# evergreen-ci/evergreen

Measured on NVIDIA H100. Metric: tasks scheduled/sec over N distros; host-allocator decisions/sec at 1/2/4/8 GPU, higher is better.
Workload: dtype int64

## Files before the change

evergreen_b200/csrc/evg_plan_general.cuh:

```cuda
#pragma once

constexpr int kGTile = 2048;

struct DGen {
  int64_t n_tiles;
  int64_t tile0;
  const int32_t* tile_distro;
  const int64_t* tile_start;
  const int64_t* dtile_off;
  unsigned long long* vmm;
  uint32_t* key_lo[2];
  uint32_t* key_hi[2];
  uint32_t* idx[2];
  uint32_t* e;
  uint32_t* tile_sum;
  uint32_t* tile_hist;
  uint4* wl;
  struct URec* pay;
  unsigned int* ccount;
  uint4* tie;
  int32_t* maxpass;
  uint32_t* run;
  uint32_t* pown;
  uint32_t* pver;
  uint32_t* pedge;
  uint32_t* sedge;
  uint32_t* rank;
  unsigned int* rcount;
  uint2* blist;
  unsigned int* bcount;
  uint4* usum;
  uint2* hlist;
  unsigned int* hcount;
  int64_t* tv;
};

__device__ __forceinline__ int gen_bits(const DGen& G, int d) {
  const unsigned long long r = G.vmm[2 * d] - G.vmm[2 * d + 1];
  return r == 0 ? 0 : 64 - __clzll((long long)r);
}
__device__ __forceinline__ int gen_npass(int bits) { return (bits + 7) >> 3; }

struct __align__(16) URec {
  int32_t prio, nd;
  int64_t exp_ns, qb;
  int32_t tgo;
  uint32_t lif;
};
static_assert(sizeof(URec) == 32, "one L2 sector per member");
constexpr uint32_t kRecGrouped = 1u << 22, kRecWaitOver = 1u << 23;
constexpr uint32_t kRunOwn = 1u << 31, kRunEntry = kRunOwn - 1u;
__device__ __forceinline__ uint32_t rec_li(const URec& r) { return r.lif & 0x1FFFFFu; }
__device__ __forceinline__ URec rec_load(const URec* p) {
  const uint4 a = reinterpret_cast<const uint4*>(p)[0], b = reinterpret_cast<const uint4*>(p)[1];
  URec r;
  r.prio = int32_t(a.x); r.nd = int32_t(a.y); r.exp_ns = int64_t((unsigned long long)a.z | ((unsigned long long)a.w << 32));
  r.qb = int64_t((unsigned long long)b.x | ((unsigned long long)b.y << 32)); r.tgo = int32_t(b.z); r.lif = b.w;
  return r;
}
__device__ __forceinline__ void rec_store(URec* p, const URec& r) {
  reinterpret_cast<uint4*>(p)[0] = make_uint4(uint32_t(r.prio), uint32_t(r.nd), uint32_t(uint64_t(r.exp_ns)), uint32_t(uint64_t(r.exp_ns) >> 32));
  reinterpret_cast<uint4*>(p)[1] = make_uint4(uint32_t(uint64_t(r.qb)), uint32_t(uint64_t(r.qb) >> 32), uint32_t(r.tgo), r.lif);
}

__global__ void k_ginit(DGen G, const int32_t* __restrict__ general_list, int n) {
  const int k = blockIdx.x * blockDim.x + threadIdx.x;
  if (k == 0) { *G.ccount = 0u; *G.maxpass = 0; *G.rcount = 0u; *G.hcount = 0u; *G.bcount = 0u; }
  if (k >= n) return;
  const int d = general_list[k];
  G.vmm[2 * d] = 0ull;
  G.vmm[2 * d + 1] = ~0ull;
}

__global__ void __launch_bounds__(256) k_gmark(DTasks T, DDistros D, DWork W, DGen G) {
  if (*W.err) return;
  const int tile = int(blockIdx.x + G.tile0);
  const int d = G.tile_distro[tile];
  const int64_t base = D.task_off[d], end = D.task_off[d + 1];
  const int64_t lo = max(G.tile_start[tile], base), hi = min(G.tile_start[tile] + kGTile, end);
  for (int64_t t = lo + threadIdx.x; t < hi; t += 256)
    for (int64_t e = T.dep_off[t]; e < T.dep_off[t + 1]; e++) W.has_dep[base + T.dep_idx[e]] = 1;
}

struct TileFold {
  unsigned int c[10];
  unsigned long long s[4];
  unsigned long long vmax, vmin;
};

constexpr int kGTaskOcc = 2;
__global__ void __launch_bounds__(256, kGTaskOcc) k_gtask(DTasks T, DDistros D, DWork W, DGen G, int64_t now, int any_complex) {
  if (*W.err) return;
  __shared__ TileFold F;
  __shared__ evg_distro_cfg s_cfg;
  __shared__ uint32_t s_nd[kNdTable];
  const int tile = int(blockIdx.x + G.tile0);
// ... 289 lines not shown
__global__ void __launch_bounds__(256, kUnitTableOcc) k_galloc(DTasks T, DDistros D, DWork W, DGen G) {
  if (*W.err) return;
  __shared__ uint32_t s_wsum[8], s_wcnt[8];
  __shared__ uint32_t s_base, s_hbase;
  const unsigned int n = *G.ccount;
  const int lane = threadIdx.x & 31, warp = threadIdx.x >> 5;
  for (unsigned int k0 = blockIdx.x * blockDim.x; k0 < n; k0 += gridDim.x * blockDim.x) {
    const unsigned int k = k0 + threadIdx.x;
    WlTask x;
    uint32_t need = 0, heads = 0;
    if (k < n) {
      x = wl_task(D, G, k);
      wl_pairs(T, G, x, k, [&](const uint32_t* place, uint32_t slot, bool) { if (*place == 0u) { need += W.unit_n[slot]; heads++; } });
    }
    uint32_t inc = need, hinc = heads;
#pragma unroll
    for (int o = 1; o < 32; o <<= 1) {
      const uint32_t y = __shfl_up_sync(0xffffffffu, inc, o), z = __shfl_up_sync(0xffffffffu, hinc, o);
      if (lane >= o) { inc += y; hinc += z; }
    }
    if (lane == 31) { s_wsum[warp] = inc; s_wcnt[warp] = hinc; }
    __syncthreads();
    uint32_t before = 0, total = 0, hbefore = 0, htotal = 0;
#pragma unroll
    for (int w = 0; w < 8; w++) {
      const uint32_t y = s_wsum[w], z = s_wcnt[w];
      before += w < warp ? y : 0u; total += y; hbefore += w < warp ? z : 0u; htotal += z;
    }
    if (threadIdx.x == 0 && htotal) { s_base = atomicAdd(G.rcount, total); s_hbase = atomicAdd(G.hcount, htotal); }
    __syncthreads();
    if (heads) {
      uint32_t pos = s_base + before + inc - need, hp = s_hbase + hbefore + hinc - heads;
      wl_pairs(T, G, x, k, [&](const uint32_t* place, uint32_t slot, bool) {
        if (*place == 0u) { W.head[slot] = pos; pos += W.unit_n[slot]; G.hlist[hp++] = make_uint2(slot, uint32_t(x.d)); }
      });
    }
    __syncthreads();
  }
}

__global__ void __launch_bounds__(256, kUnitTableOcc) k_gfill(DTasks T, DDistros D, DWork W, DGen G) {
  if (*W.err) return;
  const unsigned int n = *G.ccount;
  for (unsigned int k = blockIdx.x * blockDim.x + threadIdx.x; k < n; k += gridDim.x * blockDim.x) {
    const WlTask x = wl_task(D, G, k);
    wl_pairs(T, G, x, k, [&](const uint32_t* place, uint32_t slot, bool own) {
      G.run[W.head[slot] + *place] = k | (own ? kRunOwn : 0u);
    });
  }
}

__device__ __forceinline__ void rec_acc(UnitAcc& a, int64_t now, const URec& r) {
  acc_add(a, now, r.prio, r.exp_ns, r.qb, r.nd, (r.lif & kRecGrouped) ? 0 : -1, (r.lif >> 24) & 0x3Fu);
}
__device__ __forceinline__ bool rec_less(const URec& x, const URec& y) {
  return in_unit_less(x.tgo, x.nd, x.prio, x.exp_ns, rec_li(x), y.tgo, y.nd, y.prio, y.exp_ns, rec_li(y));
}
constexpr uint32_t kRankOne = 8;
constexpr int kRankKey = 6;

__global__ void __launch_bounds__(256, kUnitTableOcc) k_gunit(DDistros D, DWork W, DGen G, int64_t now) {
  if (*W.err) return;
  const unsigned int n = *G.hcount;
  __shared__ uint32_t s_key[kRankOne * kRankKey][256];
  for (unsigned int k = blockIdx.x * blockDim.x + threadIdx.x; k < n; k += gridDim.x * blockDim.x) {
    const uint2 u = G.hlist[k];
    const uint32_t cnt = W.unit_n[u.x], h = W.head[u.x];
    const uint32_t* run = G.run + h;
    UnitAcc a;
    acc_init(a);
    uint32_t anchor = kNoAnchor;
    const bool small = cnt <= kRankOne;
    for (uint32_t i = 0; i < cnt; i++) {
      const uint32_t q = run[i];
      const URec r = rec_load(G.pay + (q & kRunEntry));
      rec_acc(a, now, r);
      if (q & kRunOwn) anchor = min(anchor, rec_li(r));
      if (small) {
        uint32_t* kx = &s_key[i * kRankKey][threadIdx.x];
        kx[0] = uint32_t(r.tgo); kx[256] = uint32_t(r.nd); kx[512] = uint32_t(r.prio);
        kx[768] = uint32_t(uint64_t(r.exp_ns)); kx[1024] = uint32_t(uint64_t(r.exp_ns) >> 32); kx[1280] = rec_li(r);
      }
    }
    const unsigned long long v = (unsigned long long)unit_value(a, D.cfg[u.y], nullptr);
    G.usum[u.x] = make_uint4(uint32_t(v), uint32_t(v >> 32), anchor, cnt);
    W.unit_mask[u.x] = 0ull;
    if (small) {
      auto key = [&](uint32_t i, URec& r) {
        const uint32_t* kx = &s_key[i * kRankKey][threadIdx.x];
        r.tgo = int32_t(kx[0]); r.nd = int32_t(kx[256]); r.prio = int32_t(kx[512]);
        r.exp_ns = int64_t((unsigned long long)kx[768] | ((unsigned long long)kx[1024] << 32)); r.lif = kx[1280];
      };
      for (uint32_t i = 0; i < cnt; i++) {
        URec me, o;
        key(i, me);
        uint32_t rk = 0;
        for (uint32_t j = 0; j < cnt; j++) { key(j, o); rk += rec_less(o, me) ? 1u : 0u; }
        G.rank[h + i] = rk;
      }
    } else {
      const uint32_t nch = (cnt + 31) >> 5;
      const uint32_t b = atomicAdd(G.bcount, nch);
      for (uint32_t c = 0; c < nch; c++) G.blist[b + c] = make_uint2(u.x, c);
    }
  }
}

__global__ void __launch_bounds__(256, kUnitTableOcc) k_grank(DWork W, DGen G) {
  if (*W.err) return;
  const unsigned int n = *G.bcount;
  const unsigned full = 0xffffffffu;
  const int lane = threadIdx.x & 31;
  const unsigned int nw = gridDim.x * (blockDim.x >> 5);
  for (unsigned int c = blockIdx.x * (blockDim.x >> 5) + (threadIdx.x >> 5); c < n; c += nw) {
    const uint2 ch = G.blist[c];
    const uint32_t cnt = W.unit_n[ch.x], h = W.head[ch.x];
    const uint32_t* run = G.run + h;
    const uint32_t i = ch.y * 32u + uint32_t(lane);
    URec me;
    me.tgo = 0; me.nd = 0; me.prio = 0; me.exp_ns = 0; me.lif = 0;
    if (i < cnt) me = rec_load(G.pay + (run[i] & kRunEntry));
    uint32_t rk = 0;
    for (uint32_t j0 = 0; j0 < cnt; j0 += 32) {
      URec o;
      o.tgo = 0; o.nd = 0; o.prio = 0; o.exp_ns = 0; o.lif = 0;
      if (j0 + lane < cnt) o = rec_load(G.pay + (run[j0 + lane] & kRunEntry));
      const uint32_t m = min(32u, cnt - j0);
      for (uint32_t q = 0; q < m; q++) {
        URec y;
        y.tgo = __shfl_sync(full, o.tgo, q); y.nd = __shfl_sync(full, o.nd, q); y.prio = __shfl_sync(full, o.prio, q);
        y.exp_ns = __shfl_sync(full, o.exp_ns, q); y.lif = __shfl_sync(full, o.lif, q);
        rk += (i < cnt && rec_less(y, me)) ? 1u : 0u;
      }
    }
    if (i < cnt) G.rank[h + i] = rk;
  }
}

__global__ void __launch_bounds__(256, kUnitTableOcc) k_gbest(DTasks T, DDistros D, DWork W, DGen G, int want_best_pair) {
  if (*W.err) return;
  const unsigned int n = *G.ccount;
  const unsigned full = 0xffffffffu;
  const int lane = threadIdx.x & 31;
  for (unsigned int kw = blockIdx.x * blockDim.x + (threadIdx.x & ~31u); kw < n; kw += gridDim.x * blockDim.x) {
    const unsigned int k = kw + lane;
    int d = -1;
    unsigned long long kk = 0ull;
    if (k < n) {
      const WlTask x = wl_task(D, G, k);
      const uint32_t t = x.t, li = x.li;
      d = x.d;
      bool have = false;
      int64_t bv = 0;
      uint32_t ba = 0, brk = 0, bslot = kInactive, bn = 1, bkx = 0;
      if (!x.own_complex) { have = true; bv = G.tv[t]; ba = li; }
      wl_pairs(T, G, x, k, [&](const uint32_t* place, uint32_t slot, bool) {
        const uint4 u = G.usum[slot];
        const uint32_t kx = *place;
        const uint32_t a = u.z;
        if (a == kNoAnchor) return;
        const int64_t v = int64_t((unsigned long long)u.x | ((unsigned long long)u.y << 32));
        if (!have || v > bv || (v == bv && a < ba)) { have = true; bv = v; ba = a; bslot = slot; bn = u.w; bkx = kx; }
      });
      if (bslot != kInactive) {
        brk = G.rank[W.head[bslot] + bkx];
        if (bn <= 64) atomicOr(&W.unit_mask[bslot], 1ull << brk);
      }
      G.tv[t] = bv;
      G.tie[k] = make_uint4(ba, brk, bslot, 0u);
      if (want_best_pair) W.best_pair[t] = bslot;
      const bool displaced = !(ba == li && brk == 0);
      if (displaced) W.has_dep[t] |= 2;
      atomicAdd(G.e + x.base + ba, 1u);
      kk = ord_i64(bv);
    }
    const int d0 = __shfl_sync(full, d, 0);
    if (__all_sync(full, d < 0 || d == d0)) {
      unsigned long long hi = d < 0 ? 0ull : kk, lo = d < 0 ? ~0ull : kk;
#pragma unroll
      for (int o = 16; o > 0; o >>= 1) {
        hi = max(hi, __shfl_xor_sync(full, hi, o));
        lo = min(lo, __shfl_xor_sync(full, lo, o));
      }
      if (lane == 0) {
        if (hi > __ldcg(G.vmm + 2 * d0)) atomicMax(G.vmm + 2 * d0, hi);
        if (lo < __ldcg(G.vmm + 2 * d0 + 1)) atomicMin(G.vmm + 2 * d0 + 1, lo);
      }
    } else if (d >= 0) {
      if (kk > __ldcg(G.vmm + 2 * d)) atomicMax(G.vmm + 2 * d, kk);
      if (kk < __ldcg(G.vmm + 2 * d + 1)) atomicMin(G.vmm + 2 * d + 1, kk);
    }
  }
}

__global__ void k_gsched(DGen G, const int32_t* __restrict__ general_list, int n) {
  const int k = blockIdx.x * blockDim.x + threadIdx.x;
  if (k >= n) return;
  const int np = gen_npass(gen_bits(G, general_list[k]));
  if (np > 0) atomicMax(G.maxpass, np);
}

__global__ void __launch_bounds__(256) k_gsum(DDistros D, DGen G) {
  const int tile = int(blockIdx.x + G.tile0);
// ... 154 lines not shown
    uint32_t kl[8], kh[8];
#pragma unroll
    for (int m = 0; m < 8; m++) {
      const unsigned long long key = vmax_ord - ord_i64(vv[m]);
      kl[m] = uint32_t(key); kh[m] = uint32_t(key >> 32);
    }
    const uint32_t p0 = uint32_t(t8 - base);
    *reinterpret_cast<uint4*>(G.key_lo[0] + t8) = make_uint4(kl[0], kl[1], kl[2], kl[3]);
    *reinterpret_cast<uint4*>(G.key_lo[0] + t8 + 4) = make_uint4(kl[4], kl[5], kl[6], kl[7]);
    *reinterpret_cast<uint4*>(G.idx[0] + t8) = make_uint4(p0, p0 + 1, p0 + 2, p0 + 3);
    *reinterpret_cast<uint4*>(G.idx[0] + t8 + 4) = make_uint4(p0 + 4, p0 + 5, p0 + 6, p0 + 7);
    if (wide) {
      *reinterpret_cast<uint4*>(G.key_hi[0] + t8) = make_uint4(kh[0], kh[1], kh[2], kh[3]);
      *reinterpret_cast<uint4*>(G.key_hi[0] + t8 + 4) = make_uint4(kh[4], kh[5], kh[6], kh[7]);
    }
  } else {
#pragma unroll
    for (int m = 0; m < 8; m++) {
      const int64_t t = t8 + m;
      if (t >= base && t < end) gen_put(G, base, uint32_t(t - base), vmax_ord, wide, vv[m], uint32_t(t - base));
    }
  }
}

__global__ void __launch_bounds__(256) k_gplace_disp(DTasks T, DDistros D, DWork W, DGen G) {
  const unsigned int n = *G.ccount;
  for (unsigned int k = blockIdx.x * blockDim.x + threadIdx.x; k < n; k += gridDim.x * blockDim.x) {
  const uint4 ent = G.wl[k];
  const uint32_t t = ent.x;
  if (!(W.has_dep[t] & 2)) continue;
  const int d = int(ent.y);
  const int64_t base = D.task_off[d];
  const uint4 tie = G.tie[k];
  const uint32_t a = tie.x, myrk = tie.y, slot = tie.z;
  uint32_t pos = G.e[base + a];
  const uint32_t cnt = W.unit_n[slot];
  if (cnt <= 64) {
    pos += __popcll(W.unit_mask[slot] & ((1ull << myrk) - 1ull));
  } else {
    const uint32_t* run = G.run + W.head[slot];
    for (uint32_t i = 0; i < cnt; i++) {
      const uint4 tq = G.tie[run[i] & kRunEntry];
      if (tq.z == slot && tq.y < myrk) pos++;
    }
  }
  gen_put(G, base, pos, G.vmm[2 * d], gen_bits(G, d) > 32, G.tv[t], uint32_t(int64_t(t) - base));
  }
}

__device__ __forceinline__ bool gen_tile(const DDistros& D, const DGen& G, int tile, int j, int* d_out, int64_t* seg, int64_t* lo,
                                         int* cnt, bool* wide) {
  const int d = G.tile_distro[tile];
  const int bits = gen_bits(G, d);
  if (j >= gen_npass(bits)) return false;
  const int64_t base = D.task_off[d], end = D.task_off[d + 1];
  const int64_t a = max(G.tile_start[tile], base), b = min(G.tile_start[tile] + kGTile, end);
  *d_out = d; *seg = base; *lo = a; *cnt = int(b - a); *wide = bits > 32;
  return true;
}

__global__ void __launch_bounds__(256) k_ghist(int j, DDistros D, DGen G) {
  if (j >= *G.maxpass) return;
  int d, cnt; int64_t seg, lo; bool wide;
  const int tile = int(blockIdx.x + G.tile0);
  if (!gen_tile(D, G, tile, j, &d, &seg, &lo, &cnt, &wide)) return;
  const uint32_t* src = (j < 4 ? G.key_lo[j & 1] : G.key_hi[j & 1]) + lo;
  const int shift = 8 * (j & 3);
  __shared__ uint32_t h[256];
  h[threadIdx.x] = 0;
  __syncthreads();
  for (int i = threadIdx.x; i < cnt; i += 256) atomicAdd(&h[(src[i] >> shift) & 255u], 1u);
  __syncthreads();
  G.tile_hist[int64_t(tile) * 256 + threadIdx.x] = h[threadIdx.x];
}

__global__ void __launch_bounds__(1024) k_gdscan(int j, const int32_t* __restrict__ general_list, DGen G) {
// ... 156 lines not shown
```

evergreen_b200/csrc/evg_sched.cu:

```cuda
#include <cuda_runtime.h>
#include <stdarg.h>
#include <stdint.h>
#include <stdio.h>
#include <string.h>

#include <algorithm>
#include <type_traits>
#include <cstdlib>
#include <future>
#include <mutex>
#include <string>
#include <vector>

#include "evg_score.cuh"
#include "evg_intern.h"

using namespace evg;

namespace {

thread_local std::string g_err;

int fail(int code, const char* fmt, ...) {
  char buf[512];
// ... 691 lines not shown
  if (value == 0 && e != 0) {
    avg = e; sd = R.exp_std[i]; nv = e; nc = now - kMinute;
    src = EVG_DS_BACKFILL;
  } else if (since(now, coll) < ttl) {
    avg = value; sd = pstd;
    src = EVG_DS_FRESH;
  } else {
    if (doc < 0) {
      src = value == 0 ? EVG_DS_DEFAULT : EVG_DS_PREVIOUS;
      avg = value == 0 ? 10 * kMinute : value; sd = value == 0 ? 0 : pstd;
    } else {
      const int64_t a = __double2ll_rz(stat[doc].mean_ns);
      src = a == 0 ? EVG_DS_DEFAULT : EVG_DS_HISTORY;
      avg = a == 0 ? 10 * kMinute : a; sd = a == 0 ? 0 : __double2ll_rz(stat[doc].stddev_ns);
    }
    nv = avg; ns = sd; nc = now;
  }
  R.o_avg[i] = avg; R.o_std[i] = sd; R.o_value[i] = nv; R.o_pstd[i] = ns; R.o_coll[i] = nc; R.o_src[i] = src;
}

__global__ void __launch_bounds__(256) k_dur_commit(DDurRows R, const int* __restrict__ err, int64_t* __restrict__ texp,
                                                    int64_t* __restrict__ hexp, int64_t* __restrict__ hstd) {
  const int64_t i = int64_t(blockIdx.x) * blockDim.x + threadIdx.x;
  if (i >= R.n_t + R.n_h || *err) return;
  if (i < R.n_t) {
    texp[R.trows ? R.trows[i] : i] = R.o_avg[i];
  } else {
    const int64_t j = i - R.n_t, r = R.hrows ? R.hrows[j] : j;
    hexp[r] = R.o_avg[i];
    hstd[r] = R.o_std[i];
  }
}

__global__ void __launch_bounds__(256) k_breakdown(DTasks T, DDistros D, DWork W, const uint32_t* run_all, const URec* pay, int64_t now, int any_complex,
                                                   const int32_t* order, int64_t* breakdown) {
  if (*W.err) return;
  const int64_t t = int64_t(blockIdx.x) * blockDim.x + threadIdx.x;
  const int d = block_find_distro(D.task_off, D.n, t, T.n);
  if (d < 0) return;
  const int64_t base = D.task_off[d];
  const int64_t g = base + order[t];
  UnitAcc a;
  acc_init(a);
  const uint32_t bp = any_complex ? W.best_pair[g] : kInactive;
  if (bp == kInactive) {
    acc_add(a, now, T.priority[g], T.expected[g], T.qbasis[g], T.numdep[g], T.gid[g], T.flags[g]);
  } else if (W.route[d]) {
    for (uint32_t q = W.head[W.pair_slot[bp]]; q < kEnd; q = W.next[q]) {
      const uint32_t tq = pair_task(T, W, q);
      acc_add(a, now, T.priority[tq], T.expected[tq], T.qbasis[tq], T.numdep[tq], T.gid[tq], T.flags[tq]);
    }
  } else {
    const uint32_t slot = bp;
    const uint32_t* run = run_all + W.head[slot];
    const uint32_t cnt = W.unit_n[slot];
    for (uint32_t i = 0; i < cnt; i++) rec_acc(a, now, rec_load(pay + (run[i] & kRunEntry)));
  }
  int64_t bd[EVG_BD_N];
  unit_value(a, D.cfg[d], bd);
  for (int k = 0; k < EVG_BD_N; k++) breakdown[t * EVG_BD_N + k] = bd[k];
}

__global__ void k_finalize_info(DDistros D, DWork W, int32_t d_begin, int32_t d_end, int64_t g_begin, int64_t g_end) {
  int64_t i = int64_t(blockIdx.x) * blockDim.x + threadIdx.x;
  const int64_t di = d_begin + i;
  if (di < d_end && !W.route[di]) {
    evg_queue_info* q = W.qinfo + di;
    q->length = D.task_off[di + 1] - D.task_off[di];
    q->max_duration_threshold = D.cfg[di].target_time_ns;
    q->secondary_queue = q->secondary_queue != 0;
    q->has_ungrouped = q->has_ungrouped != 0;
  }
  if (g_begin + i < g_end) W.ginfo[g_begin + i].max_hosts = D.gmax[g_begin + i];
}

struct GroupScratch {
  int32_t n_hosts;
  int32_t n_free;
  double soon;
};

__device__ int eval_group(const evg_alloc_cfg& c, const evg_group_info& info, int64_t threshold, int64_t max_hosts,
                          int64_t n_hosts, int64_t n_free, double soon, int64_t* out_new, int64_t* out_free) {
  *out_new = 0;
  *out_free = 0;
  if (c.provider == EVG_PROVIDER_STATIC) return EVG_ALLOC_OK;
  if (c.has_pool) {
    if (!c.parent_found) return EVG_ALLOC_ERR_PARENT_MISSING;
    max_hosts = int64_t(c.parent_maximum_hosts) * int64_t(c.pool_max_containers);
// ... 358 lines not shown
  } dp;
  struct { DevBuf cfg, spawned, out; } hj;
  struct {
    DevBuf gmh, deps_met, gfirst, unit_max, verdict, bits, deleted, running, inert;
    DevBuf flags, est, ingest, running_db, req_off, req_group, req_ami, list, out_item, out_outcome;
    DevBuf item_off, group_off, sorted, n_sorted, unit_items, unit_off, group_id;
    DNext x{};
    std::vector<int64_t> h_item_off, h_group_off;
  } nx;
  struct { DevBuf cols, off, din, verdict, flag, pos, scan_sum, dout; } ih;
  struct { DevBuf kind, expected, dispatch, host_off, ttc, used, pos, scan_sum, pool[2], pool_off, item_off, dur, list, start, hosts_used; } es;
  DevBuf b_err;
  DevBuf b_route, b_unitv, b_unita, b_unitn, b_unitmask;
  DevBuf b_punt, b_puntcnt;
  struct RouteList {
    std::vector<int32_t> h;
    DevBuf b, lpt;
    int32_t n() const { return int32_t(h.size()); }
  };
  RouteList routes[kRoutes];
  int64_t max_cta_tasks = 0;
  int32_t nNA_big = 0;
  DevBuf b_alist;
  int64_t n_alist = 0;
  bool alist_valid = false;
  std::vector<int64_t> h_taskoff, h_groupoff, h_unitbase, h_edgeoff, h_dtileoff;
  std::vector<int32_t> h_nver;
  cudaStream_t s_h2d = nullptr, s_d2h = nullptr;
  static constexpr int kMaxChunks = 16;
  cudaEvent_t ev_h[kMaxChunks] = {}, ev_c[kMaxChunks] = {};
  int general_complex = 0;
  int64_t Tgc = 0;
  DevBuf b_kv, b_vmm, b_klo[2], b_khi[2], b_ix[2], b_e, b_tilesum, b_gmisc;
  DevBuf b_tiledistro, b_tilestart, b_dtileoff, b_tilehist, b_wl, b_pay, b_place, b_eplace, b_run, b_rank, b_blist, b_tie, b_hlist, b_usum, b_upd;
  DevBuf b_qinfo, b_ginfo, b_order, b_tv, b_bd;
  DevBuf b_hflags, b_hgid, b_hexp, b_hstd, b_hstart, b_hostoff, b_acfg, b_gs, b_result, b_status;
  bool bd_valid = false;
  evg_alloc_result* ext_result = nullptr;
  int64_t ext_capacity = 0;
  evg_alloc_result* result_ptr() const { return ext_result ? ext_result : b_result.as<evg_alloc_result>(); }
};

namespace {

DTasks dtasks(const evg_ctx* c);
DDistros ddistros(const evg_ctx* c);
DWork dwork(const evg_ctx* c);
DGen dgen(const evg_ctx* c);
inline unsigned grid_for(int64_t n, int block) { return unsigned((n + block - 1) / block); }

template <class... P, class... A>
void launch(evg_ctx* c, cudaStream_t st, void (*kernel)(P...), unsigned grid, unsigned block, size_t smem, A&&... args) {
  if (grid == 0) return;
  kernel<<<grid, block, smem, st>>>(std::forward<A>(args)...);
  c->launches++;
}

#define ENTER(c, name)                                                    \
  const char* const who = (name);                                         \
  if (!(c)) return fail(EVG_ERR_INVALID, "%s: null context", who);       \
  std::lock_guard<std::recursive_mutex> lock_((c)->mu);                   \
  CK(cudaSetDevice((c)->device))

void drop_tick(evg_ctx* c) { c->tick = {}; }

enum class Need { kTick, kOwnColumns, kEditable, kHosts, kVerdicts, kAliasMap, kDurations, kAllocated, kHostJob, kDispatchers };
int need_tick(const evg_ctx* c, const char* who, Need what) {
// ... 11 lines not shown
                      : what == Need::kDispatchers && !t.dispatchers      ? "no evg_rebuild_dispatchers on the resident tick's current run" : nullptr;
  return unmet ? fail(EVG_ERR_STATE, "%s: %s", who, unmet) : EVG_OK;
}

enum class Cols {
  kCopy,
  kChunked,
  kAdopt,
  kResident,
};

int upload_tasks(evg_ctx* c, const char* who, const evg_task_soa* t, const evg_distro_table* dt, Cols cols = Cols::kCopy,
                 const int64_t* edge_off = nullptr) {
  const bool copy_columns = cols == Cols::kCopy, adopt = cols == Cols::kAdopt;
  if (!t || !dt) return fail(EVG_ERR_INVALID, "null task table / distro table");
  const int64_t T = t->n_tasks, E = t->n_edges;
  const int32_t D = dt->n_distros;
  if (T < 0 || E < 0 || D < 0) return fail(EVG_ERR_INVALID, "negative sizes");
  if (T >= (int64_t(1) << 31) - 2) return fail(EVG_ERR_INVALID, "n_tasks %lld exceeds 2^31-2 per call", (long long)T);
  if (2 * T + E >= int64_t(0xFFFFFFF0u)) return fail(EVG_ERR_INVALID, "2*n_tasks+n_edges exceeds the 32-bit pair id space");
  if (D > 0 && (!dt->task_off || !dt->group_off || !dt->cfg)) return fail(EVG_ERR_INVALID, "null distro arrays");
  if (T > 0 && TaskCols::missing(t)) return fail(EVG_ERR_INVALID, "null task column");
  if (E > 0 && (!t->dep_off || !t->dep_idx)) return fail(EVG_ERR_INVALID, "n_edges > 0 but dep_off/dep_idx null");
  if (D == 0 && T != 0) return fail(EVG_ERR_INVALID, "tasks without distros");
  int rc = D > 0 ? check_offsets(dt->task_off, D, T, who, "task_off") : EVG_OK;
  if (rc == EVG_OK && D > 0) rc = check_offsets(dt->group_off, D, -1, who, "group_off");
  if (rc != EVG_OK) return rc;
  std::vector<int64_t> unit_base(size_t(D) + 1, 0), dtile_off(size_t(D) + 1, 0);
  std::vector<int32_t> tile_distro, list[kRoutes];
  std::vector<int64_t> tile_start;
  std::vector<uint8_t> route(size_t(D) + 1, 0);
  int general_complex = 0;
  int any_complex = E > 0 ? 1 : 0;
  int64_t Tgc = 0, Prec = 0;
  constexpr int kGA = PlanCta<kNT_A, kNCapA>::kGroupCap, kGB = PlanCta<kNT_B, kNCapB>::kGroupCap, kGC = PlanCta<kNT_C, kNCapC>::kGroupCap;
  constexpr int kBigUnits = kRoutes;
  auto size_class = [&](int32_t d) -> int {
    const int64_t a = dt->task_off[d], b = dt->task_off[d + 1];
    const int64_t n = b - a, g = dt->group_off[d + 1] - dt->group_off[d];
    const evg_distro_cfg& cf = dt->cfg[d];
    const int64_t de = (E > 0) ? (edge_off ? edge_off[d + 1] - edge_off[d] : t->dep_off[b] - t->dep_off[a]) : 0;
    const bool narrow = !cf.group_versions && de == 0;
    if (n <= kCapW) return kWarp;
    if (narrow && n <= kNCapA && g <= kGA) return kCtaA;
    if (narrow && n <= kNCapB && g <= kGB) return kCtaB;
    if (narrow && n <= kNCapC && g <= kGC) return kCtaC;
    if (n <= kCapA) return (cf.group_versions && n > kBigUnitTasks) ? kBigUnits : kSmemA;
    if (n <= kCapB) return kSmemB;
    if (n <= kCapC) return kSmemC;
    return kGeneral;
  };
  int64_t n_class[kBigUnits + 1] = {};
  for (int32_t d = 0; d < D; d++) n_class[size_class(d)]++;
  const char* sparse_env = getenv("EVG_SPARSE_CLASS");
  const int64_t sparse = sparse_env ? atoll(sparse_env) : kSparseClass;
  auto route_of = [&](int32_t d) -> int {
    const int k = size_class(d);
    if ((k == kSmemB || k == kSmemC || k == kBigUnits) && n_class[k] < sparse) return kGeneral;
    return k == kBigUnits ? kSmemA : k;
  };
  for (int32_t d = 0; d < D; d++) {
    const int64_t a = dt->task_off[d], b = dt->task_off[d + 1];
    const int64_t ga = dt->group_off[d], gb = dt->group_off[d + 1];
    if (b - a > kMaxTasksPerDistro) return fail(EVG_ERR_INVALID, "distro %d holds %lld tasks (max %lld)", d, (long long)(b - a), (long long)kMaxTasksPerDistro);
    const evg_distro_cfg& cf = dt->cfg[d];
    if (cf.n_versions < 0) return fail(EVG_ERR_INVALID, "distro %d: negative n_versions", d);
    if (gb > ga || cf.group_versions) any_complex = 1;
    unit_base[d + 1] = unit_base[d] + (gb - ga) + (cf.group_versions ? int64_t(cf.n_versions) : (b - a));
    const int64_t n = b - a;
    const int64_t de = (E > 0) ? (edge_off ? edge_off[d + 1] - edge_off[d] : t->dep_off[b] - t->dep_off[a]) : 0;
    const int r = route_of(d);
    list[r].push_back(d);
    route[d] = r != kGeneral;
    if (r == kGeneral) {
      if (gb > ga || cf.group_versions || de > 0) {
        general_complex = 1;
        Tgc += n;
        Prec += n + ((cf.group_versions && gb > ga) ? n : 0) + de;
      }
      const int64_t a0 = a & ~int64_t(3);
      for (int64_t s = a0; s < b; s += kGTile) { tile_distro.push_back(d); tile_start.push_back(s); }
    }
    dtile_off[d + 1] = int64_t(tile_distro.size());
  }
  const int64_t G = D > 0 ? dt->group_off[D] : 0;
  if (G > 0 && !dt->group_max_hosts) return fail(EVG_ERR_INVALID, "null group_max_hosts");
  const int64_t U = unit_base[D];
  if (U >= int64_t(0xFFFFFFF0u)) return fail(EVG_ERR_INVALID, "unit slot space exceeds 32 bits");
  if (Prec >= int64_t(0xFFFFFFF0u)) return fail(EVG_ERR_INVALID, "unit table exceeds 32 bits");
  if (Tgc >= int64_t(kRunOwn)) return fail(EVG_ERR_INVALID, "work list exceeds 31 bits (a run position is entry id | own bit)");
  const int64_t NT = int64_t(tile_distro.size());
  const int64_t P = 2 * T + E;
  cudaStream_t s = c->stream;
  drop_tick(c);
  if (adopt) rc = c->tasks.adopt(t);
  else if (cols != Cols::kResident) rc = c->tasks.size(T);
  if (rc == EVG_OK && copy_columns) rc = c->tasks.copy_rows(t, 0, T, s);
  if (rc != EVG_OK) return rc;
#define UPC(buf, ptr, count, type)                                                                    \
  do {                                                                                                \
    if (cols == Cols::kResident) break;                                                               \
    if (adopt) {                                                                                      \
      if ((reinterpret_cast<uintptr_t>(ptr) & 15u) != 0) return fail(EVG_ERR_INVALID, "device column %s is not 16-byte aligned", #ptr); \
      (buf).adopt(const_cast<void*>(static_cast<const void*>(ptr)));                                  \
    } else {                                                                                          \
      CK((buf).ensure(sizeof(type) * size_t((count) + kColPad)));                                     \
      if (copy_columns && (count) > 0) CK(cudaMemcpyAsync((buf).p, (ptr), sizeof(type) * size_t(count), cudaMemcpyHostToDevice, s)); \
    }                                                                                                 \
  } while (0)
  if (E > 0) {
    UPC(c->b_depoff, t->dep_off, T + 1, int64_t);
// ... 37 lines not shown
    if (on_chip) {
      CK(c->b_next.ensure(sizeof(uint32_t) * size_t(P + 1)));
      CK(c->b_pslot.ensure(sizeof(uint32_t) * size_t(P + 1)));
    }
    CK(c->b_etask.ensure(sizeof(uint32_t) * size_t(E + 1)));
    CK(c->b_elive.ensure(size_t(E) + 1));
    CK(c->b_unitv.ensure(sizeof(int64_t) * size_t(U + 1)));
    CK(c->b_unita.ensure(sizeof(uint32_t) * size_t(U + 1)));
    CK(c->b_unitn.ensure(sizeof(uint32_t) * size_t(U + 1)));
    CK(c->b_unitmask.ensure(sizeof(uint64_t) * size_t(U + 1)));
    CK(c->b_bestpair.ensure(sizeof(uint32_t) * size_t(T + 1)));
  }
  if (on_chip) CK(c->b_kv.ensure(sizeof(uint64_t) * size_t(T + 1)));
  if (!list[kGeneral].empty()) {
    for (int k = 0; k < 2; k++) {
      CK(c->b_klo[k].ensure(sizeof(uint32_t) * size_t(T + 1)));
      CK(c->b_khi[k].ensure(sizeof(uint32_t) * size_t(T + 1)));
      CK(c->b_ix[k].ensure(sizeof(uint32_t) * size_t(T + 1)));
    }
    CK(c->b_vmm.ensure(sizeof(uint64_t) * 2 * size_t(D + 1)));
    CK(c->b_gmisc.ensure(64));
    CK(c->b_tilesum.ensure(sizeof(uint32_t) * size_t(NT + 1)));
    CK(c->b_tilehist.ensure(sizeof(uint32_t) * 256 * size_t(NT + 1)));
    if (general_complex) {
      CK(c->b_e.ensure(sizeof(uint32_t) * size_t(T + kColPad)));
      CK(c->b_wl.ensure(sizeof(uint4) * size_t(Tgc + 1)));
      CK(c->b_pay.ensure(sizeof(URec) * size_t(Tgc + 1)));
      CK(c->b_tie.ensure(sizeof(uint4) * size_t(Tgc + 1)));
      CK(c->b_place.ensure(sizeof(uint32_t) * 2 * size_t(Tgc + 1)));
      CK(c->b_eplace.ensure(sizeof(uint32_t) * 2 * size_t(E + 1)));
      CK(c->b_run.ensure(sizeof(uint32_t) * size_t(Prec + 1)));
      CK(c->b_rank.ensure(sizeof(uint32_t) * size_t(Prec + 1)));
      CK(c->b_blist.ensure(sizeof(uint2) * size_t(Prec / kRankOne + 1)));
      CK(c->b_hlist.ensure(sizeof(uint2) * size_t(Prec + 1)));
      CK(c->b_usum.ensure(sizeof(uint4) * size_t(U + 1)));
    }
  }
  CK(c->b_punt.ensure(sizeof(int32_t) * size_t(D + 1)));
  CK(c->b_puntcnt.ensure(sizeof(int32_t) * (evg_ctx::kMaxChunks + 2)));
  CK(c->b_qinfo.ensure(sizeof(evg_queue_info) * size_t(D + 1)));
  CK(c->b_ginfo.ensure(sizeof(evg_group_info) * size_t(G + 1)));
  CK(c->b_order.ensure(sizeof(int32_t) * size_t(T + 1)));
  CK(c->b_tv.ensure(sizeof(int64_t) * size_t(T + kColPad)));
  c->T = T; c->E = E; c->G = G; c->U = U; c->NT = NT; c->Dn = D;
  c->t_pad = (T + 3) & ~int64_t(3);
  c->Tgc = Tgc;
  c->max_groups = 0;
  for (int32_t d = 0; d < D; d++) c->max_groups = std::max(c->max_groups, dt->group_off[d + 1] - dt->group_off[d]);
  c->any_complex = any_complex;
  c->general_complex = general_complex;
  CK(c->b_err.ensure(sizeof(int) * 4));
  CK(cudaMemsetAsync(c->b_err.p, 0, sizeof(int) * 4, s));
  for (int r = 0; r < kRoutes; r++) c->routes[r].h.swap(list[r]);
  c->h_taskoff.assign(dt->task_off, dt->task_off + D + 1);
  c->h_groupoff.assign(dt->group_off, dt->group_off + D + 1);
  c->h_edgeoff.assign(size_t(D) + 1, 0);
  if (E > 0)
    for (int32_t d = 0; d <= D; d++) c->h_edgeoff[size_t(d)] = edge_off ? edge_off[d] : t->dep_off[dt->task_off[d]];
  c->h_nver.resize(size_t(D));
  for (int32_t d = 0; d < D; d++) c->h_nver[size_t(d)] = dt->cfg[d].n_versions;
  c->h_unitbase.swap(unit_base);
  c->h_dtileoff.swap(dtile_off);
  c->tick.kind = adopt ? Tick::kBorrowed : Tick::kFixed;
  c->alist_valid = false;
  if (cols != Cols::kChunked && T > 0) {
    launch(c, s, k_validate, grid_for(T, 256), 256, 0, dtasks(c), ddistros(c), dwork(c), int64_t(0), T);
    int bad = 0;
    CK(cudaMemcpyAsync(&bad, c->b_err.p, sizeof(int), cudaMemcpyDeviceToHost, s));
// ... 56 lines not shown
  w.edge_live = c->b_elive.as<uint8_t>(); w.route = c->b_route.as<uint8_t>();
  w.err = c->b_err.as<int>();
  w.unit_v = c->b_unitv.as<int64_t>(); w.unit_a = c->b_unita.as<uint32_t>(); w.unit_n = c->b_unitn.as<uint32_t>();
  w.unit_mask = c->b_unitmask.as<unsigned long long>();
  w.best_pair = c->b_bestpair.as<uint32_t>();
  w.buf[0].key_v = c->b_kv.as<uint64_t>();
  w.qinfo = c->b_qinfo.as<evg_queue_info>(); w.ginfo = c->b_ginfo.as<evg_group_info>();
  return w;
}
DGen dgen(const evg_ctx* c) {
  DGen g;
  g.n_tiles = c->NT;
  g.tile0 = 0;
  g.tile_distro = c->b_tiledistro.as<int32_t>(); g.tile_start = c->b_tilestart.as<int64_t>();
  g.dtile_off = c->b_dtileoff.as<int64_t>();
  g.vmm = c->b_vmm.as<unsigned long long>();
  for (int k = 0; k < 2; k++) {
    g.key_lo[k] = c->b_klo[k].as<uint32_t>(); g.key_hi[k] = c->b_khi[k].as<uint32_t>(); g.idx[k] = c->b_ix[k].as<uint32_t>();
  }
  g.e = c->b_e.as<uint32_t>(); g.tile_sum = c->b_tilesum.as<uint32_t>(); g.tile_hist = c->b_tilehist.as<uint32_t>();
  g.wl = c->b_wl.as<uint4>();
  g.pay = c->b_pay.as<URec>();
  g.pown = c->b_place.as<uint32_t>();
  g.pver = c->b_place.as<uint32_t>() + (c->Tgc + 1);
  g.pedge = c->b_eplace.as<uint32_t>();
  g.sedge = c->b_eplace.as<uint32_t>() + (c->E + 1);
  g.ccount = c->b_gmisc.as<unsigned int>();
  g.maxpass = c->b_gmisc.as<int32_t>() + 1;
  g.rcount = c->b_gmisc.as<unsigned int>() + 2;
  g.hcount = c->b_gmisc.as<unsigned int>() + 3;
  g.bcount = c->b_gmisc.as<unsigned int>() + 4;
  g.blist = c->b_blist.as<uint2>();
  g.rank = c->b_rank.as<uint32_t>();
  g.hlist = c->b_hlist.as<uint2>();
  g.usum = c->b_usum.as<uint4>();
  g.run = c->b_run.as<uint32_t>();
  g.tie = c->b_tie.as<uint4>();
  g.tv = c->b_tv.as<int64_t>();
  return g;
}


int run_alloc_range(evg_ctx* c, int64_t now, int32_t d0, int32_t d1) {
  DHosts h;
  h.n = c->H; h.flags = c->b_hflags.as<uint32_t>(); h.gid = c->b_hgid.as<int32_t>();
  h.expected = c->b_hexp.as<int64_t>(); h.stddev = c->b_hstd.as<int64_t>(); h.start = c->b_hstart.as<int64_t>();
  h.host_off = c->b_hostoff.as<int64_t>(); h.cfg = c->b_acfg.as<evg_alloc_cfg>();
  if (c->ext_result && c->ext_capacity < c->Dn) return fail(EVG_ERR_INVALID, "bound result buffer holds %lld rows, need %d", (long long)c->ext_capacity, c->Dn);
  CK(c->b_gs.ensure(sizeof(GroupScratch) * size_t(c->G + 1)));
  const int split = (d1 - d0) >= 4096 ? 1 : 0;
  const bool listed = split && c->alist_valid && d0 == 0 && d1 == c->Dn;
  const int32_t* al = listed ? c->b_alist.as<int32_t>() : nullptr;
  const int64_t teams = listed ? c->n_alist : int64_t(d1 - d0);
  if (c->max_groups > kWideAllocGroups)
    launch(c, c->stream, k_alloc<128>, unsigned(teams), 128, 0, h, d0, d1, c->b_groupoff.as<int64_t>(), c->b_qinfo.as<evg_queue_info>(),
           c->b_ginfo.as<evg_group_info>(), c->b_gs.as<GroupScratch>(), now, c->result_ptr(), c->b_status.as<int32_t>(), split, al, int32_t(c->n_alist));
  else
    launch(c, c->stream, k_alloc<32>, grid_for(teams, 4), 128, 0, h, d0, d1, c->b_groupoff.as<int64_t>(), c->b_qinfo.as<evg_queue_info>(),
           c->b_ginfo.as<evg_group_info>(), c->b_gs.as<GroupScratch>(), now, c->result_ptr(), c->b_status.as<int32_t>(), split, al, int32_t(c->n_alist));
  if (split)
    launch(c, c->stream, k_alloc_groupless, grid_for(d1 - d0, 128), 128, 0, h, d0, d1, c->b_groupoff.as<int64_t>(), c->b_qinfo.as<evg_queue_info>(),
           now, c->result_ptr(), c->b_status.as<int32_t>());
  CK(cudaGetLastError());
  return EVG_OK;
}
int run_alloc(evg_ctx* c, int64_t now) { return run_alloc_range(c, now, 0, c->Dn); }

template <int THREADS, int ITEMS, int MIN_CTAS>
// ... 148 lines not shown
  }
  const std::vector<int32_t>& gh = c->routes[kGeneral].h;
  const bool general = !gh.empty();
  if (bd && c->any_complex) CK(cudaMemsetAsync(c->b_bestpair.p, 0xFF, sizeof(uint32_t) * size_t(T + 1), s));
  const int32_t n_new = bd ? 0 : c->routes[kCtaA].n() + c->routes[kCtaB].n() + c->routes[kCtaC].n();
  if (n_new > 0) CK(cudaMemsetAsync(c->b_puntcnt.p, 0, sizeof(int32_t), s));
  if (general) { int rcg = prepare_general(c, s, gh.front(), gh.back() + 1); if (rcg != EVG_OK) return rcg; }
  bool busy[evg_ctx::kAux] = {};
  for (int r = 0; r < kRoutes; r++) busy[kRouteStream[r]] |= c->routes[r].n() > 0;
  const bool fork = std::count(busy, busy + evg_ctx::kAux, true) > 1;
  if (fork) {
    int rc0 = ensure_aux_streams(c);
    if (rc0 != EVG_OK) return rc0;
    CK(cudaEventRecord(c->ev_fork, s));
    for (int k = 0; k < evg_ctx::kAux; k++) CK(cudaStreamWaitEvent(c->s_aux[k], c->ev_fork, 0));
  }
  int rc;
  const int slot = int(c->runs % evg_ctx::kRing);
  const Mode mode = bd ? Mode::kBreakdown : Mode::kResident;
  for (int r : {kCtaC, kCtaB, kCtaA, kPunted, kSmemC, kSmemB, kSmemA, kWarp, kGeneral}) {
    const int32_t n = r == kPunted ? n_new : c->routes[r].n();
    cudaStream_t sr = fork ? c->s_aux[kRouteStream[r]] : s;
    const bool time_it = c->timed && !general && c->sort_slot < 0 && n > 0 && (r == kSmemC || (r == kCtaC && !bd));
    if (time_it) CK(cudaEventRecord(c->ring0[slot], sr));
    if ((rc = plan_route(c, r, mode, sr, dt, dd, w, now, 0, n, c->b_punt.as<int32_t>(), c->b_puntcnt.as<int32_t>())) != EVG_OK) return rc;
    if (time_it) { CK(cudaEventRecord(c->ring1[slot], sr)); c->runs++; c->sort_slot = slot; }
  }
  if (fork) {
    for (int k = 0; k < evg_ctx::kAux; k++) {
      CK(cudaEventRecord(c->ev_join[k], c->s_aux[k]));
      CK(cudaStreamWaitEvent(s, c->ev_join[k], 0));
    }
  }
  if (bd) launch(c, c->stream, k_breakdown, grid_for(T, 256), 256, 0, dt, dd, w, c->b_run.as<uint32_t>(), c->b_pay.as<URec>(), now, c->any_complex, c->b_order.as<int32_t>(), bd);
  CK(cudaGetLastError());
  return EVG_OK;
}

}

extern "C" {

const char* evg_last_error(void) { return g_err.c_str(); }
int evg_abi_version(void) { return EVG_ABI_VERSION; }

int evg_init(int device, void* stream, evg_ctx** out) {
  if (!out) return fail(EVG_ERR_INVALID, "evg_init: out is null");
  *out = nullptr;
  int n = 0;
  cudaError_t e = cudaGetDeviceCount(&n);
  if (e != cudaSuccess || n == 0) return fail(EVG_ERR_CUDA, "no CUDA device: %s (libevgsched has no CPU fallback)", cudaGetErrorString(e));
  if (device < 0 || device >= n) return fail(EVG_ERR_INVALID, "device %d out of range (%d devices)", device, n);
  CK(cudaSetDevice(device));
  cudaDeviceProp prop;
  CK(cudaGetDeviceProperties(&prop, device));
  if (prop.major != 9 || prop.minor != 0)
    return fail(EVG_ERR_CUDA, "device %d is sm_%d%d; this library is built for sm_90a only", device, prop.major, prop.minor);
  evg_ctx* c = new evg_ctx();
  c->device = device;
  c->num_sms = prop.multiProcessorCount;
  if (stream) { c->stream = reinterpret_cast<cudaStream_t>(stream); c->own_stream = false; }
  else { CK(cudaStreamCreateWithFlags(&c->stream, cudaStreamNonBlocking)); c->own_stream = true; }
  CK(cudaEventCreate(&c->ev_begin)); CK(cudaEventCreate(&c->ev_sort0));
  CK(cudaEventCreate(&c->ev_sort1)); CK(cudaEventCreate(&c->ev_end));
  CK(cudaEventCreate(&c->ev_gt0)); CK(cudaEventCreate(&c->ev_gt1));
  for (int k = 0; k < evg_ctx::kRing; k++) { CK(cudaEventCreate(&c->ring0[k])); CK(cudaEventCreate(&c->ring1[k])); }
  *out = c;
// ... 2744 lines not shown
```

Baseline: 4.505 billion.

## Pack general-path unit state into compact 32-byte GUnit records indexed by head id

Replaces the per-slot unit arrays (head, usum, unit_mask, hlist) with one dense 32-byte GUnit record per unit, indexed by a compact head id. Each slot stores its id and start so later kernels read one sector. k_gfill now processes two worklist entries per thread with loads batched up front, and also rewrites the wl and edge-slot entries to unit ids. The goal is fewer scattered global reads across the fill, unit, rank and placement kernels. The cost is extra work in fill, and the diff relies on W.unit_v and on buffer sizing (Urec) that are not fully visible here.

Measured after the change: 4.836 billion (median of 6 runs). 7.4% higher.

```diff
diff --git a/evergreen_b200/csrc/evg_plan_general.cuh b/evergreen_b200/csrc/evg_plan_general.cuh
--- a/evergreen_b200/csrc/evg_plan_general.cuh
+++ b/evergreen_b200/csrc/evg_plan_general.cuh
@@ -29,8 +29,7 @@
   unsigned int* rcount;
   uint2* blist;
   unsigned int* bcount;
-  uint4* usum;
-  uint2* hlist;
+  struct GUnit* unit;
   unsigned int* hcount;
   int64_t* tv;
 };
@@ -62,6 +61,28 @@
   reinterpret_cast<uint4*>(p)[0] = make_uint4(uint32_t(r.prio), uint32_t(r.nd), uint32_t(uint64_t(r.exp_ns)), uint32_t(uint64_t(r.exp_ns) >> 32));
   reinterpret_cast<uint4*>(p)[1] = make_uint4(uint32_t(uint64_t(r.qb)), uint32_t(uint64_t(r.qb) >> 32), uint32_t(r.tgo), r.lif);
 }
+
+struct __align__(16) GUnit {
+  int64_t value;
+  uint32_t anchor;
+  uint32_t n;
+  uint32_t start;
+  int32_t d;
+  unsigned long long mask;
+};
+static_assert(sizeof(GUnit) == 32, "one L2 sector per unit");
+__device__ __forceinline__ GUnit unit_load(const GUnit* p) {
+  const uint4 a = reinterpret_cast<const uint4*>(p)[0], b = reinterpret_cast<const uint4*>(p)[1];
+  GUnit u;
+  u.value = int64_t((unsigned long long)a.x | ((unsigned long long)a.y << 32)); u.anchor = a.z; u.n = a.w;
+  u.start = b.x; u.d = int32_t(b.y); u.mask = (unsigned long long)b.z | ((unsigned long long)b.w << 32);
+  return u;
+}
+__device__ __forceinline__ void unit_store(GUnit* p, const GUnit& u) {
+  reinterpret_cast<uint4*>(p)[0] = make_uint4(uint32_t(uint64_t(u.value)), uint32_t(uint64_t(u.value) >> 32), u.anchor, u.n);
+  reinterpret_cast<uint4*>(p)[1] = make_uint4(u.start, uint32_t(u.d), uint32_t(u.mask), uint32_t(u.mask >> 32));
+}
+__device__ __forceinline__ int64_t slot_unit(uint32_t id, uint32_t start) { return int64_t(uint64_t(id) | (uint64_t(start) << 32)); }
 
 __global__ void k_ginit(DGen G, const int32_t* __restrict__ general_list, int n) {
   const int k = blockIdx.x * blockDim.x + threadIdx.x;
@@ -417,21 +438,55 @@
     if (heads) {
       uint32_t pos = s_base + before + inc - need, hp = s_hbase + hbefore + hinc - heads;
       wl_pairs(T, G, x, k, [&](const uint32_t* place, uint32_t slot, bool) {
-        if (*place == 0u) { W.head[slot] = pos; pos += W.unit_n[slot]; G.hlist[hp++] = make_uint2(slot, uint32_t(x.d)); }
+        if (*place != 0u) return;
+        GUnit u;
+        u.value = 0; u.anchor = kNoAnchor; u.n = W.unit_n[slot]; u.start = pos; u.d = x.d; u.mask = 0ull;
+        unit_store(G.unit + hp, u);
+        W.unit_v[slot] = slot_unit(hp++, pos);
+        pos += u.n;
       });
     }
     __syncthreads();
   }
 }
 
+constexpr int kFillEntries = 2;
 __global__ void __launch_bounds__(256, kUnitTableOcc) k_gfill(DTasks T, DDistros D, DWork W, DGen G) {
   if (*W.err) return;
-  const unsigned int n = *G.ccount;
-  for (unsigned int k = blockIdx.x * blockDim.x + threadIdx.x; k < n; k += gridDim.x * blockDim.x) {
-    const WlTask x = wl_task(D, G, k);
-    wl_pairs(T, G, x, k, [&](const uint32_t* place, uint32_t slot, bool own) {
-      G.run[W.head[slot] + *place] = k | (own ? kRunOwn : 0u);
-    });
+  const unsigned int n = *G.ccount, stride = gridDim.x * blockDim.x;
+  for (unsigned int k0 = blockIdx.x * blockDim.x + threadIdx.x; k0 < n; k0 += kFillEntries * stride) {
+    WlTask x[kFillEntries];
+    uint32_t place[kFillEntries][2], id[kFillEntries][2], start[kFillEntries][2];
+#pragma unroll
+    for (int j = 0; j < kFillEntries; j++) {
+      const unsigned int k = k0 + j * stride;
+      x[j].s_own = x[j].s_ver = kInactive;
+      if (k < n) x[j] = wl_task(D, G, k);
+      const uint32_t sl[2] = {x[j].s_own, x[j].s_ver};
+#pragma unroll
+      for (int m = 0; m < 2; m++) {
+        place[j][m] = sl[m] != kInactive ? (m ? G.pver : G.pown)[k] : 0u;
+        const uint64_t su = sl[m] != kInactive ? uint64_t(W.unit_v[sl[m]]) : ~0ull;
+        id[j][m] = uint32_t(su);
+        start[j][m] = uint32_t(su >> 32);
+      }
+    }
+#pragma unroll
+    for (int j = 0; j < kFillEntries; j++) {
+      const unsigned int k = k0 + j * stride;
+      if (k >= n) continue;
+      if (id[j][0] != kInactive) G.run[start[j][0] + place[j][0]] = k | kRunOwn;
+      if (id[j][1] != kInactive) G.run[start[j][1] + place[j][1]] = k;
+      G.wl[k] = make_uint4(x[j].t, uint32_t(x[j].d), id[j][0], id[j][1]);
+      if (T.n_edges > 0)
+        for (int64_t e = T.dep_off[x[j].t]; e < T.dep_off[x[j].t + 1]; e++) {
+          const uint32_t sl = G.sedge[e];
+          if (sl == kInactive) continue;
+          const uint64_t su = uint64_t(W.unit_v[sl]);
+          G.run[uint32_t(su >> 32) + G.pedge[e]] = k;
+          G.sedge[e] = uint32_t(su);
+        }
+    }
   }
 }
 
@@ -449,8 +504,8 @@
   const unsigned int n = *G.hcount;
   __shared__ uint32_t s_key[kRankOne * kRankKey][256];
   for (unsigned int k = blockIdx.x * blockDim.x + threadIdx.x; k < n; k += gridDim.x * blockDim.x) {
-    const uint2 u = G.hlist[k];
-    const uint32_t cnt = W.unit_n[u.x], h = W.head[u.x];
+    GUnit u = unit_load(G.unit + k);
+    const uint32_t cnt = u.n, h = u.start;
     const uint32_t* run = G.run + h;
     UnitAcc a;
     acc_init(a);
@@ -467,9 +522,10 @@
         kx[768] = uint32_t(uint64_t(r.exp_ns)); kx[1024] = uint32_t(uint64_t(r.exp_ns) >> 32); kx[1280] = rec_li(r);
       }
     }
-    const unsigned long long v = (unsigned long long)unit_value(a, D.cfg[u.y], nullptr);
-    G.usum[u.x] = make_uint4(uint32_t(v), uint32_t(v >> 32), anchor, cnt);
-    W.unit_mask[u.x] = 0ull;
+    u.value = unit_value(a, D.cfg[u.d], nullptr);
+    u.anchor = anchor;
+    u.mask = 0ull;
+    unit_store(G.unit + k, u);
     if (small) {
       auto key = [&](uint32_t i, URec& r) {
         const uint32_t* kx = &s_key[i * kRankKey][threadIdx.x];
@@ -486,7 +542,7 @@
     } else {
       const uint32_t nch = (cnt + 31) >> 5;
       const uint32_t b = atomicAdd(G.bcount, nch);
-      for (uint32_t c = 0; c < nch; c++) G.blist[b + c] = make_uint2(u.x, c);
+      for (uint32_t c = 0; c < nch; c++) G.blist[b + c] = make_uint2(k, c);
     }
   }
 }
@@ -499,7 +555,8 @@
   const unsigned int nw = gridDim.x * (blockDim.x >> 5);
   for (unsigned int c = blockIdx.x * (blockDim.x >> 5) + (threadIdx.x >> 5); c < n; c += nw) {
     const uint2 ch = G.blist[c];
-    const uint32_t cnt = W.unit_n[ch.x], h = W.head[ch.x];
+    const GUnit u = unit_load(G.unit + ch.x);
+    const uint32_t cnt = u.n, h = u.start;
     const uint32_t* run = G.run + h;
     const uint32_t i = ch.y * 32u + uint32_t(lane);
     URec me;
@@ -537,23 +594,23 @@
       d = x.d;
       bool have = false;
       int64_t bv = 0;
-      uint32_t ba = 0, brk = 0, bslot = kInactive, bn = 1, bkx = 0;
+      uint32_t ba = 0, brk = 0, bid = kInactive, bn = 1, bpos = 0;
       if (!x.own_complex) { have = true; bv = G.tv[t]; ba = li; }
-      wl_pairs(T, G, x, k, [&](const uint32_t* place, uint32_t slot, bool) {
-        const uint4 u = G.usum[slot];
+      wl_pairs(T, G, x, k, [&](const uint32_t* place, uint32_t id, bool) {
+        const GUnit u = unit_load(G.unit + id);
         const uint32_t kx = *place;
-        const uint32_t a = u.z;
-        if (a == kNoAnchor) return;
-        const int64_t v = int64_t((unsigned long long)u.x | ((unsigned long long)u.y << 32));
-        if (!have || v > bv || (v == bv && a < ba)) { have = true; bv = v; ba = a; bslot = slot; bn = u.w; bkx = kx; }
+        if (u.anchor == kNoAnchor) return;
+        if (!have || u.value > bv || (u.value == bv && u.anchor < ba)) {
+          have = true; bv = u.value; ba = u.anchor; bid = id; bn = u.n; bpos = u.start + kx;
+        }
       });
-      if (bslot != kInactive) {
-        brk = G.rank[W.head[bslot] + bkx];
-        if (bn <= 64) atomicOr(&W.unit_mask[bslot], 1ull << brk);
+      if (bid != kInactive) {
+        brk = G.rank[bpos];
+        if (bn <= 64) atomicOr(&G.unit[bid].mask, 1ull << brk);
       }
       G.tv[t] = bv;
-      G.tie[k] = make_uint4(ba, brk, bslot, 0u);
-      if (want_best_pair) W.best_pair[t] = bslot;
+      G.tie[k] = make_uint4(ba, brk, bid, 0u);
+      if (want_best_pair) W.best_pair[t] = bid;
       const bool displaced = !(ba == li && brk == 0);
       if (displaced) W.has_dep[t] |= 2;
       atomicAdd(G.e + x.base + ba, 1u);
@@ -774,16 +831,16 @@
   const int d = int(ent.y);
   const int64_t base = D.task_off[d];
   const uint4 tie = G.tie[k];
-  const uint32_t a = tie.x, myrk = tie.y, slot = tie.z;
+  const uint32_t a = tie.x, myrk = tie.y, id = tie.z;
   uint32_t pos = G.e[base + a];
-  const uint32_t cnt = W.unit_n[slot];
-  if (cnt <= 64) {
-    pos += __popcll(W.unit_mask[slot] & ((1ull << myrk) - 1ull));
+  const GUnit u = unit_load(G.unit + id);
+  if (u.n <= 64) {
+    pos += __popcll(u.mask & ((1ull << myrk) - 1ull));
   } else {
-    const uint32_t* run = G.run + W.head[slot];
-    for (uint32_t i = 0; i < cnt; i++) {
+    const uint32_t* run = G.run + u.start;
+    for (uint32_t i = 0; i < u.n; i++) {
       const uint4 tq = G.tie[run[i] & kRunEntry];
-      if (tq.z == slot && tq.y < myrk) pos++;
+      if (tq.z == id && tq.y < myrk) pos++;
     }
   }
   gen_put(G, base, pos, G.vmm[2 * d], gen_bits(G, d) > 32, G.tv[t], uint32_t(int64_t(t) - base));
diff --git a/evergreen_b200/csrc/evg_sched.cu b/evergreen_b200/csrc/evg_sched.cu
--- a/evergreen_b200/csrc/evg_sched.cu
+++ b/evergreen_b200/csrc/evg_sched.cu
@@ -747,8 +747,8 @@
   }
 }
 
-__global__ void __launch_bounds__(256) k_breakdown(DTasks T, DDistros D, DWork W, const uint32_t* run_all, const URec* pay, int64_t now, int any_complex,
-                                                   const int32_t* order, int64_t* breakdown) {
+__global__ void __launch_bounds__(256) k_breakdown(DTasks T, DDistros D, DWork W, const uint32_t* run_all, const URec* pay, const GUnit* units,
+                                                   int64_t now, int any_complex, const int32_t* order, int64_t* breakdown) {
   if (*W.err) return;
   const int64_t t = int64_t(blockIdx.x) * blockDim.x + threadIdx.x;
   const int d = block_find_distro(D.task_off, D.n, t, T.n);
@@ -766,10 +766,9 @@
       acc_add(a, now, T.priority[tq], T.expected[tq], T.qbasis[tq], T.numdep[tq], T.gid[tq], T.flags[tq]);
     }
   } else {
-    const uint32_t slot = bp;
-    const uint32_t* run = run_all + W.head[slot];
-    const uint32_t cnt = W.unit_n[slot];
-    for (uint32_t i = 0; i < cnt; i++) rec_acc(a, now, rec_load(pay + (run[i] & kRunEntry)));
+    const GUnit u = unit_load(units + bp);
+    const uint32_t* run = run_all + u.start;
+    for (uint32_t i = 0; i < u.n; i++) rec_acc(a, now, rec_load(pay + (run[i] & kRunEntry)));
   }
   int64_t bd[EVG_BD_N];
   unit_value(a, D.cfg[d], bd);
@@ -1194,7 +1193,7 @@
   int general_complex = 0;
   int64_t Tgc = 0;
   DevBuf b_kv, b_vmm, b_klo[2], b_khi[2], b_ix[2], b_e, b_tilesum, b_gmisc;
-  DevBuf b_tiledistro, b_tilestart, b_dtileoff, b_tilehist, b_wl, b_pay, b_place, b_eplace, b_run, b_rank, b_blist, b_tie, b_hlist, b_usum, b_upd;
+  DevBuf b_tiledistro, b_tilestart, b_dtileoff, b_tilehist, b_wl, b_pay, b_place, b_eplace, b_run, b_rank, b_blist, b_tie, b_unit, b_upd;
   DevBuf b_qinfo, b_ginfo, b_order, b_tv, b_bd;
   DevBuf b_hflags, b_hgid, b_hexp, b_hstd, b_hstart, b_hostoff, b_acfg, b_gs, b_result, b_status;
   bool bd_valid = false;
@@ -1272,7 +1271,7 @@
   std::vector<uint8_t> route(size_t(D) + 1, 0);
   int general_complex = 0;
   int any_complex = E > 0 ? 1 : 0;
-  int64_t Tgc = 0, Prec = 0;
+  int64_t Tgc = 0, Prec = 0, Urec = 0;
   constexpr int kGA = PlanCta<kNT_A, kNCapA>::kGroupCap, kGB = PlanCta<kNT_B, kNCapB>::kGroupCap, kGC = PlanCta<kNT_C, kNCapC>::kGroupCap;
   constexpr int kBigUnits = kRoutes;
   auto size_class = [&](int32_t d) -> int {
@@ -1317,6 +1316,7 @@
         general_complex = 1;
         Tgc += n;
         Prec += n + ((cf.group_versions && gb > ga) ? n : 0) + de;
+        Urec += n + ((cf.group_versions && gb > ga) ? std::min<int64_t>(cf.n_versions, n) : 0);
       }
       const int64_t a0 = a & ~int64_t(3);
       for (int64_t s = a0; s < b; s += kGTile) { tile_distro.push_back(d); tile_start.push_back(s); }
@@ -1420,8 +1420,7 @@
       CK(c->b_run.ensure(sizeof(uint32_t) * size_t(Prec + 1)));
       CK(c->b_rank.ensure(sizeof(uint32_t) * size_t(Prec + 1)));
       CK(c->b_blist.ensure(sizeof(uint2) * size_t(Prec / kRankOne + 1)));
-      CK(c->b_hlist.ensure(sizeof(uint2) * size_t(Prec + 1)));
-      CK(c->b_usum.ensure(sizeof(uint4) * size_t(U + 1)));
+      CK(c->b_unit.ensure(sizeof(GUnit) * size_t(Urec + 1)));
     }
   }
   CK(c->b_punt.ensure(sizeof(int32_t) * size_t(D + 1)));
@@ -1544,8 +1543,7 @@
   g.bcount = c->b_gmisc.as<unsigned int>() + 4;
   g.blist = c->b_blist.as<uint2>();
   g.rank = c->b_rank.as<uint32_t>();
-  g.hlist = c->b_hlist.as<uint2>();
-  g.usum = c->b_usum.as<uint4>();
+  g.unit = c->b_unit.as<GUnit>();
   g.run = c->b_run.as<uint32_t>();
   g.tie = c->b_tie.as<uint4>();
   g.tv = c->b_tv.as<int64_t>();
@@ -1760,7 +1758,7 @@
       CK(cudaStreamWaitEvent(s, c->ev_join[k], 0));
     }
   }
-  if (bd) launch(c, c->stream, k_breakdown, grid_for(T, 256), 256, 0, dt, dd, w, c->b_run.as<uint32_t>(), c->b_pay.as<URec>(), now, c->any_complex, c->b_order.as<int32_t>(), bd);
+  if (bd) launch(c, c->stream, k_breakdown, grid_for(T, 256), 256, 0, dt, dd, w, c->b_run.as<uint32_t>(), c->b_pay.as<URec>(), c->b_unit.as<GUnit>(), now, c->any_complex, c->b_order.as<int32_t>(), bd);
   CK(cudaGetLastError());
   return EVG_OK;
 }
```
